# sgl-project/rbg

Hardware: NVIDIA B200
Metric: replica_x_node_affinity_scores_per_sec (higher is better)
Workload: dtype f32

## Files before the change

rbg_b200/csrc/plan_group.cuh:

```cuda
#pragma once
#include "select_fast.cuh"

namespace rbgtopo {

struct GroupTab {
  int* node;
  int* cons;
  float* aw;
  int mask, HT;
  int* cnt;
  int* dSlot;
  float* dBase;
  int* dFree;
  int* dAvail;
  int* dDom;
};
struct GroupRole {
  int count, demand, need, flags;
};

__host__ __device__ inline size_t group_smem_bytes(int QB, int PB, int HT, int CAP) {
  return (size_t)HT * 4 * (2 + QB) + (size_t)CAP * 20 +
         (size_t)PB * KS * (3 * 8 + 3 * 4) +
         (size_t)MAXP * 16 + (size_t)MAXP * RBGTOPO_MAX_GROUP_ROLES * 4;
}

__device__ __forceinline__ int gtab_insert(const GroupTab& T, int n) {
  int h = tab_hash(n, T.mask);
  while (true) {
    const int old = atomicCAS(&T.node[h], -1, n);
    if (old == -1) T.dSlot[atomicAdd(T.cnt, 1)] = h;
    if (old == -1 || old == n) return h;
    h = (h + 1) & T.mask;
  }
}
__device__ __forceinline__ bool gtab_has(const GroupTab& T, int n) {
  int h = tab_hash(n, T.mask);
  while (true) {
    const int k = T.node[h];
    if (k == n) return true;
    if (k == -1) return false;
    h = (h + 1) & T.mask;
  }
}
__device__ __forceinline__ float gtab_delta(const GroupTab& T, const float* pair_row, int Q, int slot) {
  float d = 0.0f;
  const float* aw = T.aw + slot;
  for (int q = 0; q < Q; ++q, aw += T.HT) d = fmaf(pair_row[q], *aw, d);
  return d;
}

#ifdef RBGTOPO_PHASE_CLOCKS
__device__ long long g_phase_clk[2048 * 32];
__device__ int g_dbg_skip;
__device__ long long g_cta_ns[2048 * 4];
__device__ __forceinline__ long long pg_gtime() { long long t; asm volatile("mov.u64 %0, %%globaltimer;" : "=l"(t)); return t; }
__device__ __forceinline__ int pg_smid() { int v; asm volatile("mov.u32 %0, %%smid;" : "=r"(v)); return v; }
#define PCLK(k) do { if (tid == 0 && blockIdx.x < 2048 && (k) < 32) g_phase_clk[blockIdx.x * 32 + (k)] = clock64(); } while (0)
#define PCLKL(k) do { if ((k) >= 0 && (threadIdx.x & 31) == 0 && blockIdx.x < 2048 && (k) < 32) g_phase_clk[blockIdx.x * 32 + (k)] = clock64(); } while (0)
#else
#define PCLK(k) do {} while (0)
#define PCLKL(k) do {} while (0)
#endif

struct BgCand {
  unsigned long long ob;
  int node, free_, owner, dom;
};
__device__ __forceinline__ BgCand bg_attrs(const TopoDev& t, int need_i, int i, int n_sel, unsigned long long ob) {
  BgCand c;
  c.ob = ob;
  c.node = -1;
  c.free_ = 0;
  c.owner = -1;
  c.dom = -1;
  if (i < n_sel) {
    c.node = need_i > 0 ? key_node(ob) : i;
    c.free_ = t.free_[c.node];
    c.owner = t.node_owner[c.node];
    c.dom = t.domain[c.node];
  }
  return c;
}
__device__ __forceinline__ BgCand bg_load(const TopoDev& t, int need_i, int i, int n_sel) {
  return bg_attrs(t, need_i, i, n_sel, (i < n_sel && need_i > 0) ? t.order_all[i] : 0ull);
}

__device__ __forceinline__ void select_role_group(const TopoDev& t, int gid, bool excl_step, const GroupRole& role,
                                                  const float* pair_row, int Q, int K, int dom, const GroupTab& T,
                                                  int cnt, bool have_first, const BgCand& first, int dbg,
                                                  unsigned long long* sAcc, int* sAccAv,
                                                  unsigned long long* sPat, int* sPatAv, unsigned long long* out,
                                                  int* outAvail) {
  const int lane = threadIdx.x & 31;
  if (dom == DOM_NONE || K <= 0) {
    out[lane] = 0;
    outAvail[lane] = 0;
    __syncwarp();
    return;
  }
  const int demand = role.demand;
  const float need = (float)role.need;
  const bool rexcl = excl_step && (role.flags & RBGTOPO_ROLE_EXCLUSIVE);

  constexpr int EREG = 8;
  auto entry_key = [&](int i) -> unsigned long long {
    const int av = T.dAvail[i], dd = T.dDom[i];
    if (av >= demand && !(rexcl && dd < 0) && (dom == DOM_ANY || (dd & 0x7FFFFFFF) == dom)) {
      const int slot = T.dSlot[i];
      return make_key(fmaf(need, T.dBase[i], gtab_delta(T, pair_row, Q, slot)), T.node[slot]);
    }
    return 0ull;
  };
  unsigned long long kreg[EREG];
#ifdef RBGTOPO_PHASE_CLOCKS
  if (g_dbg_skip & 2) cnt = 0;
#endif
#pragma unroll
  for (int j = 0; j < EREG; ++j) {
    kreg[j] = 0ull;
    if (32 * j < cnt) {
      const int i = lane + 32 * j;
      if (i < cnt) kreg[j] = entry_key(i);
    }
  }
  int npat = 0;
  {
    unsigned long long prev = ~0ull;
    for (; npat < K; ++npat) {
      unsigned long long best = 0;
      int bi = 0;
#pragma unroll
      for (int j = 0; j < EREG; ++j)
        if (32 * j < cnt && kreg[j] < prev && kreg[j] > best) { best = kreg[j]; bi = lane + 32 * j; }
      for (int i = lane + 32 * EREG; i < cnt; i += 32) {
        const unsigned long long k = entry_key(i);
        if (k < prev && k > best) { best = k; bi = i; }
      }
      const unsigned long long m = warp_max_u64(best);
      if (m == 0) break;
      if (best == m) { sPat[npat] = m; sPatAv[npat] = T.dAvail[bi]; }
      prev = m;
    }
  }
  __syncwarp();
  PCLKL(dbg);

  int acc = 0;
  for (int pos = 0; pos < t.n && acc < K; pos += 32) {
    const BgCand c = (pos == 0 && have_first) ? first : bg_load(t, role.need, pos + lane, t.n);
    bool ok = c.node >= 0 && c.free_ >= demand;
    if (ok && rexcl) ok = (c.owner == -1 || c.owner == gid);
    if (ok && dom != DOM_ANY) ok = c.dom == dom;
    if (ok) ok = !gtab_has(T, c.node);
    const uint32_t m = __ballot_sync(FULL, ok);
    const int idx = acc + __popc(m & ((1u << lane) - 1u));
    if (ok && idx < K) {
      const float base = __uint_as_float((uint32_t)(c.ob >> 32) ^ 0x80000000u);
      sAcc[idx] = role.need > 0 ? make_key(need * base, c.node) : make_key(0.0f, c.node);
      sAccAv[idx] = c.free_;
    }
    acc += __popc(m);
  }
  acc = min(acc, K);
  __syncwarp();
  PCLKL(dbg < 0 ? -1 : dbg + 1);

  merge_lists(sAcc, sAccAv, acc, sPat, sPatAv, npat, K, out, outAvail);
}

__device__ __forceinline__ void gtab_add_anchor(const TopoDev& t, const GroupTab& T, int m, int q, int c, int dem) {
  const int lane = threadIdx.x & 31;
  if (lane == 0 && dem > 0) atomicAdd(&T.cons[gtab_insert(T, m)], dem);
  if (c <= 0) return;
  const int rb = t.row_ptr[m], re = t.row_ptr[m + 1];
  for (int j = rb + lane; j <= re; j += 32) {
    int nn, wv;
    if (j < re) {
      nn = t.col[j];
      wv = t.w[j] * c;
    } else {
      nn = m;
      wv = RBGTOPO_SELF_W * c;
    }
    atomicAdd(&T.aw[(size_t)q * T.HT + gtab_insert(T, nn)], (float)wv);
  }
}

__device__ __forceinline__ int wave_next(const int* roles, int q, int& cr, int& taken, int* role, int* count) {
  while (cr < q && roles[4 * cr + 1] - taken <= 0) { ++cr; taken = 0; }
  if (cr >= q) return 0;
  const int level = roles[4 * cr];
  int n = 0, P = 0;
  while (cr < q && roles[4 * cr] == level && n < RBGTOPO_MAX_STEP_REPLICAS && P < RBGTOPO_MAX_STEP_ROLES) {
    const int left = roles[4 * cr + 1] - taken;
    if (left <= 0) { ++cr; taken = 0; continue; }
    const int take = min(left, RBGTOPO_MAX_STEP_REPLICAS - n);
    role[P] = cr;
    count[P] = take;
    ++P;
    n += take;
    taken += take;
    if (taken == roles[4 * cr + 1]) { ++cr; taken = 0; }
  }
  return P;
}

constexpr int RTAB_WARPS = 4;
__global__ void __launch_bounds__(32 * RTAB_WARPS) k_group_rtab(const int* __restrict__ grp, int words, int n_groups, int n_rows,
                                                              int2* __restrict__ rtab) {
  __shared__ int sR[RTAB_WARPS][4 * RBGTOPO_MAX_GROUP_ROLES], sP[RTAB_WARPS][RBGTOPO_MAX_GROUP_ROLES * RBGTOPO_MAX_GROUP_ROLES];
  __shared__ int sPl[RTAB_WARPS][RBGTOPO_MAX_GROUP_ROLES], sRole[RTAB_WARPS][RBGTOPO_MAX_STEP_ROLES], sCount[RTAB_WARPS][RBGTOPO_MAX_STEP_ROLES];
  __shared__ int sRec[RTAB_WARPS][RBGTOPO_MAX_STEP_ROLES], sNP[RTAB_WARPS];
  const int lane = threadIdx.x & 31, wi = threadIdx.x >> 5;
  const int g = blockIdx.x * RTAB_WARPS + wi;
  if (g >= n_groups) return;
  const int* rec = grp + RBGTOPO_HDR_WORDS + (size_t)g * RBGTOPO_GROUP_WORDS;
  const int gid = rec[0], q = rec[3];
  const long long roff = rec[4], poff = rec[5];
  const bool excl = (rec[1] & RBGTOPO_STEP_EXCLUSIVE) != 0;
  if (q < 1 || q > RBGTOPO_MAX_GROUP_ROLES || roff < 0 || roff + 4 * q > words || poff < 0 || poff + q * q > words) return;
  if (rec[9] <= 0) return;
  for (int i = lane; i < 4 * q; i += 32) sR[wi][i] = grp[roff + i];
  for (int i = lane; i < q * q; i += 32) sP[wi][i] = grp[poff + i];
  if (lane < RBGTOPO_MAX_GROUP_ROLES) sPl[wi][lane] = 0;
  __syncwarp();
  int cr = 0, tk = 0;
  long long row = rec[8];
  if (row < 0) return;
  while (row < n_rows) {
    if (lane == 0) sNP[wi] = wave_next(sR[wi], q, cr, tk, sRole[wi], sCount[wi]);
    __syncwarp();
    const int P = sNP[wi];
    if (P == 0) break;
    if (lane < P) {
      const int ri = sRole[wi][lane];
      int need = 0;
      for (int j = 0; j < q; ++j)
        if (sP[wi][ri * q + j] > 0) need += sR[wi][4 * j + 1] - sPl[wi][j];
      const bool rexcl = excl && (sR[wi][4 * ri + 3] & RBGTOPO_ROLE_EXCLUSIVE);
      sRec[wi][lane] = emit_pack_row(sR[wi][4 * ri + 2], max(0, min(need, RBGTOPO_NEED_CAP)), rexcl);
    }
    __syncwarp();
    for (int p = 0; p < P; ++p) {
      const int cnt = sCount[wi][p];
      const int2 rr = make_int2(sRec[wi][p], gid);
      if (lane < cnt && row + lane < n_rows) rtab[row + lane] = rr;
      row += cnt;
    }
    if (lane < P) sPl[wi][sRole[wi][lane]] += sCount[wi][lane];
    __syncwarp();
  }
}

template <bool DIRECT>
__global__ void __launch_bounds__(32 * MAXP, 4) k_plan_group(TopoDev t, BatchDev b, int QB, int HT, int CAP, int record) {
  extern __shared__ __align__(16) unsigned char pg_smem[];
  __shared__ int sTakenNode[KS], sTakenAmt[KS], sTakenRole[KS], sRowB[KS], sRowN[KS];
  __shared__ int sDstar, sCnt, sNew, sStatus, sAny, sCorrN;
  const int tid = threadIdx.x, warp = tid >> 5, lane = tid & 31, nthreads = blockDim.x, nwarps = nthreads >> 5;
  const int PB = nwarps;
  GroupTab T;
  T.node = reinterpret_cast<int*>(pg_smem);
  T.cons = T.node + HT;
  T.aw = reinterpret_cast<float*>(T.cons + HT);
  T.mask = HT - 1;
  T.HT = HT;
  T.cnt = &sCnt;
  T.dSlot = reinterpret_cast<int*>(T.aw + (size_t)QB * HT);
  T.dBase = reinterpret_cast<float*>(T.dSlot + CAP);
  T.dFree = reinterpret_cast<int*>(T.dBase + CAP);
  T.dAvail = T.dFree + CAP;
  T.dDom = T.dAvail + CAP;
  unsigned long long* sList = reinterpret_cast<unsigned long long*>(T.dDom + CAP);
  unsigned long long* sAcc = sList + (size_t)PB * KS;
  unsigned long long* sPat = sAcc + (size_t)PB * KS;
  int* sListAv = reinterpret_cast<int*>(sPat + (size_t)PB * KS);
  int* sAccAv = sListAv + (size_t)PB * KS;
  int* sPatAv = sAccAv + (size_t)PB * KS;
  GroupRole* sRole = reinterpret_cast<GroupRole*>(sPatAv + (size_t)PB * KS);
  float* sPair = reinterpret_cast<float*>(sRole + MAXP);

  if (record) pdl_launch_dependents();
  PCLK(30);
#ifdef RBGTOPO_PHASE_CLOCKS
  if (tid == 0 && blockIdx.x < 2048) { g_cta_ns[blockIdx.x * 4] = pg_gtime(); g_cta_ns[blockIdx.x * 4 + 3] = pg_smid(); }
#endif
  int wave_i = 0;
  int step = b.perm ? b.perm[blockIdx.x] : blockIdx.x;
  __shared__ int sGR[DIRECT ? 4 * RBGTOPO_MAX_GROUP_ROLES : 1];
  __shared__ int sGP[DIRECT ? RBGTOPO_MAX_GROUP_ROLES * RBGTOPO_MAX_GROUP_ROLES : 1];
  __shared__ int sPlaced[DIRECT ? RBGTOPO_MAX_GROUP_ROLES : 1];
  __shared__ int sWRole[DIRECT ? RBGTOPO_MAX_STEP_ROLES : 1], sWCount[DIRECT ? RBGTOPO_MAX_STEP_ROLES : 1];
  __shared__ int sWP, sWN, sCr, sTk;
  int g_rep0 = 0, g_pend = 0, g_i0 = 0, g_stat = 0, g_dom = -1;
  StepHdr h;
  if (DIRECT) {
    const int* rec = b.blob + RBGTOPO_HDR_WORDS + (size_t)step * RBGTOPO_GROUP_WORDS;
    h.gid = rec[0];
    h.flags = rec[1] & (RBGTOPO_STEP_EXCLUSIVE | RBGTOPO_STEP_GANG);
    h.fixed_domain = (rec[1] & RBGTOPO_STEP_EXCLUSIVE) ? rec[2] : -1;
    h.Q = rec[3];
    h.role_off = rec[4];
    h.pair_off = rec[5];
    h.n_anchors = rec[6];
    h.anchor_off = rec[7];
    h.i0 = 0;
    g_rep0 = rec[8];
    g_pend = rec[9];
    h.P = 0; h.R = 0; h.rep_off = g_rep0; h.rolerow_off = 0; h.next_step = 0; h.n_cons = 0; h.cons_off = 0;
  } else {
    h = load_hdr(b, step);
  }
  for (int i = tid; i < HT; i += nthreads) {
    T.node[i] = -1;
    T.cons[i] = 0;
  }
  for (int i = tid; i < QB * HT; i += nthreads) T.aw[i] = 0.0f;
  if (tid == 0) sCnt = 0;
  if (DIRECT) {
    for (int i = tid; i < 4 * h.Q; i += nthreads) sGR[i] = b.blob[h.role_off + i];
    for (int i = tid; i < h.Q * h.Q; i += nthreads) sGP[i] = b.blob[h.pair_off + i];
    if (tid < RBGTOPO_MAX_GROUP_ROLES) sPlaced[tid] = 0;
    if (tid == 0) { sCr = 0; sTk = 0; }
  }
  const bool excl_step = (h.flags & RBGTOPO_STEP_EXCLUSIVE) != 0;
  const bool gang = (h.flags & RBGTOPO_STEP_GANG) != 0;
  const int gid = h.gid, Q = h.Q;
  int fixed = excl_step ? h.fixed_domain : -1;
  g_dom = fixed;
  const size_t stride = (size_t)t.slab_stride;
  __syncthreads();

  {
    const int* anc = b.blob + h.anchor_off;
    for (int a = warp; a < h.n_anchors - h.i0; a += nwarps) gtab_add_anchor(t, T, anc[3 * a], anc[3 * a + 1], anc[3 * a + 2], 0);
  }
  int n_new = 0;
  int cnt_done = 0;

  while (true) {
    PCLK(wave_i * 8 + 0);
    const unsigned long long ob0 = lane < t.n ? t.order_all[lane] : 0ull;
    if (DIRECT) {
      if (tid == 0) {
        int cr = sCr, tk = sTk;
        const int P = wave_next(sGR, Q, cr, tk, sWRole, sWCount);
        int n = 0;
        for (int k = 0; k < P; ++k) n += sWCount[k];
        sCr = cr;
        sTk = tk;
        sWP = P;
        sWN = n;
      }
      __syncthreads();
      h.P = sWP;
      h.R = sWN;
      h.rep_off = g_rep0 + g_i0;
      if (h.P == 0) break;
      if (tid < h.P) {
        const int ri = sWRole[tid];
        int need = 0;
        for (int j = 0; j < Q; ++j)
          if (sGP[ri * Q + j] > 0) need += sGR[4 * j + 1] - sPlaced[j];
        sRole[tid] = GroupRole{sWCount[tid], sGR[4 * ri + 2], min(need, RBGTOPO_NEED_CAP), (sGR[4 * ri + 3] & 0xFF) | (ri << 8)};
      }
      for (int i = tid; i < h.P * Q; i += nthreads)
        sPair[(i / Q) * RBGTOPO_MAX_GROUP_ROLES + i % Q] = (float)sGP[sWRole[i / Q] * Q + i % Q];
    } else {
      if (tid < h.P) {
        const int4 r = *reinterpret_cast<const int4*>(b.blob + h.role_off + 4 * tid);
        sRole[tid] = GroupRole{r.x, r.y, r.z, r.w};
      }
      for (int i = tid; i < h.P * Q; i += nthreads)
        sPair[(i / Q) * RBGTOPO_MAX_GROUP_ROLES + i % Q] = (float)b.blob[h.pair_off + i];
    }
    if (tid == 0) sCorrN = 0;
    if (tid < n_new) {
      const int m = sTakenNode[tid];
      const int rb = t.row_ptr[m], re = t.row_ptr[m + 1];
      sRowB[tid] = rb;
      sRowN[tid] = re - rb + 1;
      atomicAdd(&T.cons[gtab_insert(T, m)], sTakenAmt[tid]);
    }
    __syncthreads();
    BgCand first;
    const bool have_first = warp < h.P;
    if (have_first) first = bg_attrs(t, sRole[warp].need, lane, t.n, ob0);
    {
      int total = 0;
      for (int a = 0; a < n_new; ++a) total += sRowN[a];
      for (int e = tid; e < total; e += nthreads) {
        int a = 0, off = e;
        while (off >= sRowN[a]) off -= sRowN[a++];
        const int m = sTakenNode[a], q = sTakenRole[a];
        int nn, wv;
        if (off < sRowN[a] - 1) {
          nn = t.col[sRowB[a] + off];
          wv = t.w[sRowB[a] + off];
        } else {
          nn = m;
          wv = RBGTOPO_SELF_W;
        }
        atomicAdd(&T.aw[(size_t)q * HT + gtab_insert(T, nn)], (float)wv);
      }
    }
    __syncthreads();
    PCLK(wave_i * 8 + 1);

    const int cnt = sCnt;
    for (int d = cnt_done + tid; d < cnt; d += nthreads) {
      const int node = T.node[T.dSlot[d]];
      int dd = t.domain[node];
      if (excl_step) {
        const int o = t.node_owner[node];
        if (!(o == -1 || o == gid)) dd |= 0x80000000;
      }
      T.dBase[d] = t.base[node];
      T.dFree[d] = t.free_[node];
      T.dDom[d] = dd;
    }
    cnt_done = cnt;
    __syncthreads();
    for (int d = tid; d < cnt; d += nthreads) T.dAvail[d] = T.dFree[d] - T.cons[T.dSlot[d]];
    __syncthreads();
    PCLK(wave_i * 8 + 2);

    PCLK(wave_i * 8 + 3);
    int dstar = excl_step ? fixed : -1;
    if (excl_step && fixed < 0) {
      int pstar = -1;
      for (int p = 0; p < h.P; ++p)
        if (sRole[p].flags & RBGTOPO_ROLE_EXCLUSIVE) { pstar = p; break; }
      if (warp == 0) {
        int d = -1;
        if (pstar >= 0) {
          select_role_group(t, gid, excl_step, sRole[pstar], sPair + pstar * RBGTOPO_MAX_GROUP_ROLES, Q, 1, DOM_ANY, T,
                            cnt, pstar == 0, first, 29, sAcc, sAccAv, sPat, sPatAv, sList, sListAv);
          const unsigned long long top = sList[0];
          d = top ? t.domain[key_node(top)] : -1;
        }
        if (lane == 0) sDstar = d;
      }
      __syncthreads();
      dstar = sDstar;
    }
    if (warp < h.P) {
      const int p = warp;
      const bool rexcl = excl_step && (sRole[p].flags & RBGTOPO_ROLE_EXCLUSIVE);
      const int dom = rexcl ? (dstar >= 0 ? dstar : DOM_NONE) : DOM_ANY;
      int K = 0;
      for (int q = 0; q <= p; ++q) K += sRole[q].count;
      K = min(K, t.n);
      select_role_group(t, gid, excl_step, sRole[p], sPair + p * RBGTOPO_MAX_GROUP_ROLES, Q, K, dom, T, cnt, true, first, warp == 0 ? wave_i * 8 + 6 : -1,
                        sAcc + p * KS, sAccAv + p * KS, sPat + p * KS, sPatAv + p * KS, sList + p * KS,
                        sListAv + p * KS);
      if (!DIRECT) b.merged[(size_t)(h.rolerow_off + p) * KS + lane] = sList[p * KS + lane];
    }
    __syncthreads();
    PCLK(wave_i * 8 + 4);

#ifdef RBGTOPO_PHASE_CLOCKS
    if (!(g_dbg_skip & 1))
#endif
    if (warp != 0 && record) {
      int* const reg = b.corr + (size_t)b.poff[step] * b.corr_w;
      for (int d = tid - 32; d < cnt; d += nthreads - 32) {
        const int slot = T.dSlot[d];
        const int node = T.node[slot];
        if (node < t.slab_lo || node >= t.slab_hi) continue;
        const int av = T.dAvail[d];
        const bool consumed = T.cons[slot] > 0;
        float v[MAXP];
        bool any = false;
#pragma unroll
        for (int p = 0; p < MAXP; ++p) {
          v[p] = 0.0f;
          if (p < h.P) {
            v[p] = (consumed && av < sRole[p].demand) ? -INFINITY
                                                      : gtab_delta(T, sPair + p * RBGTOPO_MAX_GROUP_ROLES, Q, slot);
            any |= v[p] != 0.0f;
          }
        }
        if (any) {
          int* e = reg + (size_t)atomicAdd(&sCorrN, 1) * b.corr_w;
          e[0] = node;
#pragma unroll
          for (int p = 0; p < MAXP; ++p)
            if (p < h.P) e[1 + p] = __float_as_int(v[p]);
        }
      }
    } else if (warp != 0) {
      if (wave_i == 0) {
        pdl_wait();
        pdl_launch_dependents();
      }
      float* const mrow0 = b.matrix + (size_t)h.rep_off * stride - t.slab_lo;
      for (int d = tid - 32; d < cnt; d += nthreads - 32) {
        const int slot = T.dSlot[d];
        const int node = T.node[slot];
        if (node < t.slab_lo || node >= t.slab_hi) continue;
        const int av = T.dAvail[d];
        const bool consumed = T.cons[slot] > 0;
        float* rowp = mrow0 + node;
        for (int p = 0; p < h.P; ++p) {
          const int count = sRole[p].count;
          if (consumed && av < sRole[p].demand) {
            for (int k = 0; k < count; ++k) rowp[(size_t)k * stride] = -INFINITY;
          } else {
            const float add = gtab_delta(T, sPair + p * RBGTOPO_MAX_GROUP_ROLES, Q, slot);
            if (add != 0.0f)
              for (int k = 0; k < count; ++k) sel_red_add_f32(rowp + (size_t)k * stride, add);
          }
          rowp += (size_t)count * stride;
        }
      }
    }

    if (warp == 0) {
      int tnode = -1, tamt = 0, trole = 0;
      int ntaken = 0, unplaced = 0, r = 0;
      for (int p = 0; p < h.P; ++p) {
        const int count = sRole[p].count, demand = sRole[p].demand;
        const int grole = (sRole[p].flags >> 8) & 0xFF;
        const unsigned long long key = sList[p * KS + lane];
        const int node = key ? key_node(key) : -1;
        const int av = sListAv[p * KS + lane];
        for (int c = 0; c < count; ++c, ++r) {
          int used = 0;
          for (int i = 0; i < ntaken; ++i) {
            const int n_i = __shfl_sync(FULL, tnode, i), a_i = __shfl_sync(FULL, tamt, i);
            used += n_i == node ? a_i : 0;
          }
          const uint32_t okm = __ballot_sync(FULL, key != 0 && av - used >= demand);
          const int pick = okm ? __shfl_sync(FULL, node, __ffs(okm) - 1) : -1;
          if (pick >= 0) {
            if (lane == ntaken) { tnode = pick; tamt = demand; trole = grole; }
            ++ntaken;
          } else {
            ++unplaced;
          }
          if (lane == 0) b.assign[h.rep_off + r] = pick;
        }
      }
      int status = unplaced ? RBGTOPO_PLACED_PART : RBGTOPO_PLACED_ALL;
      if (unplaced && gang) {
        status = RBGTOPO_GANG_FAILED;
        for (int i = lane; i < h.R; i += 32) b.assign[h.rep_off + i] = -1;
        ntaken = 0;
      }
      if (lane < ntaken) {
        sTakenNode[lane] = tnode;
        sTakenAmt[lane] = tamt;
        sTakenRole[lane] = trole;
      }
      if (lane == 0) {
        if (!DIRECT) {
          b.status[step] = status;
          b.domain_out[step] = dstar;
          b.dstar[step] = dstar;
        }
        sNew = ntaken;
        sStatus = status;
        sAny = ntaken > 0;
      }
    }
    if (DIRECT && tid < h.P) sPlaced[sWRole[tid]] += sWCount[tid];
    __syncthreads();
    if (record && tid == 0) b.corr_cnt[step] = sCorrN;
    PCLK(wave_i * 8 + 5);
    ++wave_i;
    if (DIRECT) {
      g_stat = max(g_stat, sStatus);
      if (dstar >= 0) g_dom = dstar;
      g_i0 += h.R;
      n_new = sNew;
      if (excl_step && dstar >= 0 && sAny) fixed = dstar;
      if (sStatus == RBGTOPO_GANG_FAILED) break;
      continue;
    }
    if (h.next_step <= 0) break;
    n_new = sNew;
    if (excl_step && dstar >= 0 && sAny) fixed = dstar;
    if (sStatus == RBGTOPO_GANG_FAILED) {
      if (warp == 0)
        for (int s2 = h.next_step; s2 > 0;) {
          const StepHdr h2 = load_hdr(b, s2);
          for (int i = lane; i < h2.R; i += 32) b.assign[h2.rep_off + i] = -1;
          if (lane == 0) {
            b.status[s2] = RBGTOPO_GANG_FAILED;
            b.domain_out[s2] = -1;
            b.dstar[s2] = -1;
            if (record) b.corr_cnt[s2] = 0;
          }
          s2 = h2.next_step;
        }
      break;
    }
    step = h.next_step;
    h = load_hdr(b, step);
  }
  if (DIRECT) {
    if (g_stat == RBGTOPO_GANG_FAILED || (gang && g_stat != RBGTOPO_PLACED_ALL)) {
      for (int i = tid; i < g_pend; i += nthreads) b.assign[g_rep0 + i] = -1;
      g_stat = RBGTOPO_GANG_FAILED;
      g_dom = -1;
    }
    if (tid == 0) {
      b.status[step] = g_stat;
      b.domain_out[step] = excl_step ? g_dom : -1;
    }
  }
  PCLK(31);
#ifdef RBGTOPO_PHASE_CLOCKS
  if (tid == 0 && blockIdx.x < 2048) { g_cta_ns[blockIdx.x * 4 + 1] = pg_gtime(); g_cta_ns[blockIdx.x * 4 + 2] = sCnt; }
#endif
}

constexpr int CORRECT_WARPS = 4;
__global__ void __launch_bounds__(32 * CORRECT_WARPS) k_plan_correct(TopoDev t, BatchDev b) {
  const int lane = threadIdx.x & 31;
  const int step = blockIdx.x * CORRECT_WARPS + (threadIdx.x >> 5);
  if (step >= b.n_steps) return;
  const int cnt = b.corr_cnt[step];
  if (cnt <= 0) return;
  const int* __restrict__ hdr = b.blob + RBGTOPO_HDR_WORDS + (size_t)step * RBGTOPO_STEP_WORDS;
  const int P = hdr[3], role_off = hdr[4], rep_off = hdr[12];
  const int my_count = lane < P ? b.blob[role_off + 4 * lane] : 0;
  const size_t stride = (size_t)t.slab_stride;
  float* const mrow0 = b.matrix + (size_t)rep_off * stride - t.slab_lo;
  const int* const reg = b.corr + (size_t)b.poff[step] * b.corr_w;
  for (int e0 = 0; e0 < cnt; e0 += 32) {
    const int e = e0 + lane;
    const int* rec = reg + (size_t)e * b.corr_w;
    float* rowp = e < cnt ? mrow0 + rec[0] : nullptr;
    for (int p = 0; p < P; ++p) {
      const int count = __shfl_sync(FULL, my_count, p);
      if (e < cnt) {
        const float v = __int_as_float(rec[1 + p]);
        if (v == -INFINITY) {
          for (int k = 0; k < count; ++k) rowp[(size_t)k * stride] = -INFINITY;
        } else if (v != 0.0f) {
          for (int k = 0; k < count; ++k) sel_red_add_f32(rowp + (size_t)k * stride, v);
        }
        rowp += (size_t)count * stride;
      }
    }
  }
}

}
```

rbg_b200/csrc/select.cuh:

```cuda
#pragma once
#include "kernels.cuh"
#include "p2p.cuh"

namespace rbgtopo {

constexpr int DOM_ANY = -2;
constexpr int DOM_NONE = -1;

constexpr int STEP_SKIP = 4;
constexpr int SEL_CORRECT = 1;
constexpr int SEL_CHAIN = 2;

struct StepHdr {
  int gid, flags, fixed_domain, P, role_off, Q, pair_off, n_anchors, anchor_off, n_cons, cons_off, R, rep_off,
      rolerow_off, next_step, i0;
};
__device__ __forceinline__ StepHdr load_hdr(const BatchDev& b, int step) {
  const int* hdr = b.blob + RBGTOPO_HDR_WORDS + (size_t)step * RBGTOPO_STEP_WORDS;
  StepHdr h;
  h.gid = hdr[0]; h.flags = hdr[1]; h.fixed_domain = hdr[2]; h.P = hdr[3]; h.role_off = hdr[4];
  h.Q = hdr[5]; h.pair_off = hdr[6]; h.n_anchors = hdr[7]; h.anchor_off = hdr[8];
  h.n_cons = hdr[9]; h.cons_off = hdr[10]; h.R = hdr[11]; h.rep_off = hdr[12]; h.rolerow_off = hdr[13];
  h.next_step = hdr[14]; h.i0 = hdr[15];
  return h;
}
__device__ __forceinline__ int role_k(const BatchDev& b, const StepHdr& h, int p, int n) {
  int k = 0;
  for (int q = 0; q <= p; ++q) k += b.blob[h.role_off + 4 * q];
  return min(k, n);
}
__device__ __forceinline__ int role_rowbase(const BatchDev& b, const StepHdr& h, int p) {
  int k = 0;
  for (int q = 0; q < p; ++q) k += b.blob[h.role_off + 4 * q];
  return k;
}

__device__ __forceinline__ void build_candidates(const TopoDev& t, const BatchDev& b, const StepHdr& h,
                                                 int* cand, int* sCnt) {
  const int lane = threadIdx.x & 31, warp = threadIdx.x >> 5, nwarps = blockDim.x >> 5;
  const int* anc = b.blob + h.anchor_off;
  for (int a = warp; a < h.n_anchors; a += nwarps) {
    const int m = anc[3 * a];
    const int rb = t.row_ptr[m], re = t.row_ptr[m + 1];
    for (int j0 = rb; j0 <= re; j0 += 32) {
      const int j = j0 + lane;
      int nn = -1;
      if (j < re) nn = t.col[j];
      else if (j == re) nn = m;
      const bool keep = nn >= t.slab_lo && nn < t.slab_hi;
      const uint32_t msk = __ballot_sync(FULL, keep);
      int base = 0;
      if (lane == 0 && msk) base = atomicAdd(sCnt, __popc(msk));
      base = __shfl_sync(FULL, base, 0);
      if (keep) cand[base + __popc(msk & ((1u << lane) - 1u))] = nn;
    }
  }
  const int* con = b.blob + h.cons_off;
  for (int c = threadIdx.x; c < h.n_cons; c += blockDim.x) {
    const int m = con[2 * c];
    if (m >= t.slab_lo && m < t.slab_hi) cand[atomicAdd(sCnt, 1)] = m;
  }
}

__device__ __forceinline__ void sel_red_add_f32(float* p, float v) {
  asm volatile("red.global.add.f32 [%0], %1;" ::"l"(p), "f"(v) : "memory");
}

__device__ __forceinline__ void correct_step(const TopoDev& t, const BatchDev& b, const StepHdr& h) {
  const int lane = threadIdx.x & 31, warp = threadIdx.x >> 5, nwarps = blockDim.x >> 5;
  const size_t stride = (size_t)t.slab_stride;
  float* const mrow0 = b.matrix + (size_t)h.rep_off * stride - t.slab_lo;
  const int* con = b.blob + h.cons_off;
  for (int c = threadIdx.x; c < h.n_cons; c += blockDim.x) {
    const int m = con[2 * c];
    if (m >= t.slab_lo && m < t.slab_hi && con[2 * c + 1] > 0) {
      int amt = 0;
      for (int k = 0; k < h.n_cons; ++k)
        if (con[2 * k] == m) amt += con[2 * k + 1];
      const int avail = t.free_[m] - amt;
      float* rowp = mrow0 + m;
      for (int p = 0; p < h.P; ++p) {
        const int count = b.blob[h.role_off + 4 * p], demand = b.blob[h.role_off + 4 * p + 1];
        if (avail < demand)
          for (int k = 0; k < count; ++k) rowp[(size_t)k * stride] = -INFINITY;
        rowp += (size_t)count * stride;
      }
    }
  }
  const int* anc = b.blob + h.anchor_off;
  for (int a = warp; a < h.n_anchors; a += nwarps) {
    const int m = anc[3 * a], q = anc[3 * a + 1], c = anc[3 * a + 2];
    if (c == 0) continue;
    const int rb = t.row_ptr[m], re = t.row_ptr[m + 1];
    for (int j = rb + lane; j <= re; j += 32) {
      int nn, wv;
      if (j < re) {
        nn = t.col[j];
        wv = t.w[j] * c;
      } else {
        nn = m;
        wv = RBGTOPO_SELF_W * c;
      }
      if (nn >= t.slab_lo && nn < t.slab_hi) {
        float* rowp = mrow0 + nn;
        for (int p = 0; p < h.P; ++p) {
          const int count = b.blob[h.role_off + 4 * p];
          const int coef = b.blob[h.pair_off + p * h.Q + q];
          if (coef) {
            const float add = (float)(coef * wv);
            for (int k = 0; k < count; ++k) sel_red_add_f32(rowp + (size_t)k * stride, add);
          }
          rowp += (size_t)count * stride;
        }
      }
    }
  }
}

__device__ __forceinline__ void select_role(const TopoDev& t, const BatchDev& b, const StepHdr& h, int p,
                                            int K, int dom, const int* cand, int cnt,
                                            unsigned long long* kcache, int kcap,
                                            unsigned long long* sAcc, unsigned long long* sPat,
                                            unsigned long long* out) {
  const int lane = threadIdx.x & 31;
  if (dom == DOM_NONE || K <= 0) {
    out[lane] = 0;
    return;
  }
  const int demand = b.blob[h.role_off + 4 * p + 1];
  const int need_i = b.blob[h.role_off + 4 * p + 2];
  const bool rexcl = (h.flags & RBGTOPO_STEP_EXCLUSIVE) && (b.blob[h.role_off + 4 * p + 3] & RBGTOPO_ROLE_EXCLUSIVE);
  const float* __restrict__ row =
      b.matrix + (size_t)(h.rep_off + role_rowbase(b, h, p)) * t.slab_stride - t.slab_lo;

  int npat = 0;
  {
    const bool cached = kcache != nullptr && cnt <= kcap;
    if (cached) {
      for (int i = lane; i < cnt; i += 32) {
        const int node = cand[i];
        const float x = row[node];
        kcache[i] = (x != -INFINITY && (dom == DOM_ANY || t.domain[node] == dom)) ? make_key(x, node) : 0ull;
      }
      __syncwarp();
    }
    unsigned long long prev = ~0ull;
    for (; npat < K; ++npat) {
      unsigned long long best = 0;
      if (cached) {
        for (int i = lane; i < cnt; i += 32) {
          const unsigned long long k = kcache[i];
          if (k < prev && k > best) best = k;
        }
      } else {
        for (int i = lane; i < cnt; i += 32) {
          const int node = cand[i];
          const float x = row[node];
          if (x != -INFINITY && (dom == DOM_ANY || t.domain[node] == dom)) {
            const unsigned long long k = make_key(x, node);
            if (k < prev && k > best) best = k;
          }
        }
      }
      best = warp_max_u64(best);
      if (best == 0) break;
      if (lane == 0) sPat[npat] = best;
      prev = best;
    }
  }

  const int slab_len = t.slab_hi - t.slab_lo;
  const float need = (float)need_i;
  int acc = 0;
  for (int pos = 0; pos < slab_len && acc < K; pos += 32) {
    const int i = pos + lane;
    int node = -1;
    unsigned long long key = 0;
    bool ok = false;
    if (i < slab_len) {
      if (need_i > 0) {
        const unsigned long long ob = t.order[i];
        node = key_node(ob);
        const float base = __uint_as_float((uint32_t)(ob >> 32) ^ 0x80000000u);
        key = make_key(need * base, node);
      } else {
        node = t.slab_lo + i;
        key = make_key(0.0f, node);
      }
      ok = t.free_[node] >= demand;
      if (ok && rexcl) {
        const int o = t.node_owner[node];
        ok = (o == -1 || o == h.gid);
      }
      if (ok && dom != DOM_ANY) ok = t.domain[node] == dom;
    }
    if (__any_sync(FULL, ok)) {
      for (int e = 0; e < cnt; ++e)
        if (cand[e] == node) ok = false;
    }
    const uint32_t m = __ballot_sync(FULL, ok);
    const int idx = acc + __popc(m & ((1u << lane) - 1u));
    if (ok && idx < K) sAcc[idx] = key;
    acc += __popc(m);
  }
  acc = min(acc, K);
  __syncwarp();

  if (lane == 0) {
    int ia = 0, ip = 0;
    for (int r = 0; r < KS; ++r) {
      unsigned long long v = 0;
      if (r < K) {
        const unsigned long long a = ia < acc ? sAcc[ia] : 0ull;
        const unsigned long long c = ip < npat ? sPat[ip] : 0ull;
        if (a > c) { v = a; ++ia; } else if (c) { v = c; ++ip; }
      }
      out[r] = v;
    }
  }
  __syncwarp();
}

__device__ __forceinline__ void chain_step(const BatchDev& b, const StepHdr& h, int status, int dstar) {
  const int lane = threadIdx.x & 31;
  __syncwarp();
  int* wb = const_cast<int*>(b.blob);
  const bool excl = (h.flags & RBGTOPO_STEP_EXCLUSIVE) != 0;
  const bool dead = status == RBGTOPO_GANG_FAILED;
  bool any = false;
  for (int i = 0; i < h.R; ++i) any |= b.assign[h.rep_off + i] >= 0;
  const int fixed = excl ? ((dstar >= 0 && any) ? dstar : h.fixed_domain) : -1;
  for (int s2 = h.next_step; s2 > 0;) {
    int* hd = wb + RBGTOPO_HDR_WORDS + (size_t)s2 * RBGTOPO_STEP_WORDS;
    const int n_static = hd[7] - hd[15];
    int rr = 0;
    for (int p = 0; p < h.P; ++p) {
      const int count = b.blob[h.role_off + 4 * p], demand = b.blob[h.role_off + 4 * p + 1];
      const int q = (b.blob[h.role_off + 4 * p + 3] >> 8) & 0xFF;
      for (int c = lane; c < count; c += 32) {
        const int node = b.assign[h.rep_off + rr + c];
        int* ar = wb + hd[8] + 3 * (n_static + h.i0 + rr + c);
        int* cr = wb + hd[10] + 2 * (h.i0 + rr + c);
        ar[0] = node >= 0 ? node : 0;
        ar[1] = q;
        ar[2] = node >= 0 ? 1 : 0;
        cr[0] = node >= 0 ? node : 0;
        cr[1] = node >= 0 ? demand : 0;
      }
      rr += count;
    }
    const int nxt = hd[14];
    if (lane == 0) {
      hd[2] = fixed;
      hd[1] = dead ? (hd[1] | STEP_SKIP) : (hd[1] & ~STEP_SKIP);
    }
    s2 = nxt;
  }
}

__device__ __forceinline__ void greedy_step(const TopoDev& t, const BatchDev& b, int step, const StepHdr& h,
                                            const unsigned long long (*sList)[KS], int* sTakenNode,
                                            int* sTakenAmt, int dstar, bool chain = false) {
  const int lane = threadIdx.x & 31;
  const int* con = b.blob + h.cons_off;
  int ntaken = 0, unplaced = 0, r = 0;
  for (int p = 0; p < h.P; ++p) {
    const int count = b.blob[h.role_off + 4 * p], demand = b.blob[h.role_off + 4 * p + 1];
    for (int c = 0; c < count; ++c, ++r) {
      int pick = -1;
      for (int k = 0; k < KS; ++k) {
        const unsigned long long key = sList[p][k];
        if (key == 0) break;
        const int node = key_node(key);
        int used = 0;
        for (int i = lane; i < h.n_cons; i += 32)
          if (con[2 * i] == node) used += con[2 * i + 1];
        for (int i = lane; i < ntaken; i += 32)
          if (sTakenNode[i] == node) used += sTakenAmt[i];
        used = __reduce_add_sync(FULL, used);
        if (t.free_[node] - used >= demand) {
          pick = node;
          break;
        }
      }
      if (pick >= 0) {
        if (lane == 0) {
          sTakenNode[ntaken] = pick;
          sTakenAmt[ntaken] = demand;
        }
        ++ntaken;
        __syncwarp();
      } else {
        ++unplaced;
      }
      if (lane == 0) b.assign[h.rep_off + r] = pick;
    }
  }
  __syncwarp();
  int status = unplaced ? RBGTOPO_PLACED_PART : RBGTOPO_PLACED_ALL;
  if (unplaced && (h.flags & RBGTOPO_STEP_GANG)) {
    status = RBGTOPO_GANG_FAILED;
    for (int i = lane; i < h.R; i += 32) b.assign[h.rep_off + i] = -1;
  }
  if (lane == 0) {
    b.status[step] = status;
    b.domain_out[step] = dstar;
    b.dstar[step] = dstar;
  }
  if (chain && h.next_step > 0) chain_step(b, h, status, dstar);
}

constexpr int CAND_CAP = 512;
__host__ __device__ inline size_t select_smem_bytes(int PB) { return (size_t)CAND_CAP * 4 + (size_t)PB * CAND_CAP * 8; }

struct CandRef { const int* p; int cnt; };
__device__ __forceinline__ CandRef stage_candidates(const TopoDev& t, const BatchDev& b, int step, const StepHdr& h,
                                                    int* sCand, int* sCnt) {
  const int cap = b.poff[step + 1] - b.poff[step];
  int* dst = cap <= CAND_CAP ? sCand : b.cand + b.poff[step];
  if (threadIdx.x == 0) *sCnt = 0;
  __syncthreads();
  build_candidates(t, b, h, dst, sCnt);
  __syncthreads();
  CandRef r;
  r.p = dst;
  r.cnt = *sCnt;
  return r;
}

__global__ void __launch_bounds__(32 * MAXP) k_select_assign(TopoDev t, BatchDev b, int step_begin, int mode) {
  extern __shared__ __align__(16) unsigned char sel_smem[];
  int* sCand = reinterpret_cast<int*>(sel_smem);
  unsigned long long* sKeys = reinterpret_cast<unsigned long long*>(sel_smem + (size_t)CAND_CAP * 4);
  __shared__ unsigned long long sList[MAXP][KS];
  __shared__ unsigned long long sAcc[MAXP][KS];
  __shared__ unsigned long long sPat[MAXP][KS];
  __shared__ int sTakenNode[KS], sTakenAmt[KS];
  __shared__ int sDstar, sCnt;
  const int warp = threadIdx.x >> 5, lane = threadIdx.x & 31;
  const int step = step_begin + blockIdx.x;
  const StepHdr h = load_hdr(b, step);
  const bool excl_step = (h.flags & RBGTOPO_STEP_EXCLUSIVE) != 0;
  if (h.flags & STEP_SKIP) {
    if (warp == 0) {
      for (int i = lane; i < h.R; i += 32) b.assign[h.rep_off + i] = -1;
      if (lane == 0) {
        b.status[step] = RBGTOPO_GANG_FAILED;
        b.domain_out[step] = -1;
        b.dstar[step] = -1;
      }
    }
    return;
  }
  if (mode & SEL_CORRECT) {
    correct_step(t, b, h);
    __threadfence();
  }
  const CandRef cr = stage_candidates(t, b, step, h, sCand, &sCnt);
  const int* cand = cr.p;
  const int cnt = cr.cnt;
  int dstar = excl_step ? h.fixed_domain : -1;
  if (excl_step && h.fixed_domain < 0) {
    int pstar = -1;
    for (int p = 0; p < h.P; ++p)
      if (b.blob[h.role_off + 4 * p + 3] & RBGTOPO_ROLE_EXCLUSIVE) { pstar = p; break; }
    if (warp == 0) {
      int d = -1;
      if (pstar >= 0) {
        select_role(t, b, h, pstar, 1, DOM_ANY, cand, cnt, sKeys, CAND_CAP, sAcc[0], sPat[0], sList[0]);
        const unsigned long long top = sList[0][0];
        d = top ? t.domain[key_node(top)] : -1;
      }
      if (lane == 0) sDstar = d;
    }
    __syncthreads();
    dstar = sDstar;
  }
  if (warp < h.P) {
    const int p = warp;
    const bool rexcl = excl_step && (b.blob[h.role_off + 4 * p + 3] & RBGTOPO_ROLE_EXCLUSIVE);
    const int dom = rexcl ? (dstar >= 0 ? dstar : DOM_NONE) : DOM_ANY;
    select_role(t, b, h, p, role_k(b, h, p, t.n), dom, cand, cnt, sKeys + (size_t)p * CAND_CAP, CAND_CAP, sAcc[p],
                sPat[p], sList[p]);
    b.merged[(size_t)(h.rolerow_off + p) * KS + lane] = sList[p][lane];
  }
  __syncthreads();
  if (warp == 0) greedy_step(t, b, step, h, sList, sTakenNode, sTakenAmt, dstar, (mode & SEL_CHAIN) != 0);
}

__global__ void __launch_bounds__(32 * MAXP) k_select(TopoDev t, BatchDev b, int pass2) {
  extern __shared__ __align__(16) unsigned char sel_smem[];
  int* sCand = reinterpret_cast<int*>(sel_smem);
  unsigned long long* sKeys = reinterpret_cast<unsigned long long*>(sel_smem + (size_t)CAND_CAP * 4);
  __shared__ unsigned long long sAcc[MAXP][KS];
  __shared__ unsigned long long sPat[MAXP][KS];
  __shared__ int sCnt;
  const int warp = threadIdx.x >> 5;
  const int step = blockIdx.x;
  const StepHdr h = load_hdr(b, step);
  const bool excl_step = (h.flags & RBGTOPO_STEP_EXCLUSIVE) != 0;
  const bool unknown = excl_step && h.fixed_domain < 0;
  if (pass2 && !unknown) return;
  const CandRef cr = stage_candidates(t, b, step, h, sCand, &sCnt);
  const int* cand = cr.p;
  const int cnt = cr.cnt;
  if (warp >= h.P) return;
  const int p = warp;
  const bool rexcl = excl_step && (b.blob[h.role_off + 4 * p + 3] & RBGTOPO_ROLE_EXCLUSIVE);
  const int K = role_k(b, h, p, t.n);
  if (!pass2) {
    const int dom = (rexcl && !unknown) ? h.fixed_domain : DOM_ANY;
    select_role(t, b, h, p, K, dom, cand, cnt, sKeys + (size_t)p * CAND_CAP, CAND_CAP, sAcc[p], sPat[p],
                b.lists + (size_t)(h.rolerow_off + p) * KS);
  } else if (rexcl) {
    const int d = b.dstar[step];
    select_role(t, b, h, p, K, d >= 0 ? d : DOM_NONE, cand, cnt, sKeys + (size_t)p * CAND_CAP, CAND_CAP, sAcc[p],
                sPat[p], b.excl + (size_t)(h.rolerow_off + p) * KS);
  }
}

constexpr int SEL_WARPS = 4;
constexpr int SEL_THREADS = SEL_WARPS * 32;

__device__ __forceinline__ int merge_parts(const unsigned long long* src, long long stride, int parts, int K,
                                           unsigned long long* out ) {
  const int lane = threadIdx.x & 31;
  unsigned long long prev = ~0ull;
  int r = 0;
  for (; r < K; ++r) {
    unsigned long long best = 0;
    for (int i = lane; i < parts * K; i += 32) {
      const unsigned long long k = src[(long long)(i / K) * stride + (i % K)];
      if (k < prev && k > best) best = k;
    }
    best = warp_max_u64(best);
    if (best == 0) break;
    if (lane == 0) out[r] = best;
    prev = best;
  }
  for (int q = r + lane; q < KS; q += 32) out[q] = 0;
  __syncwarp();
  return r;
}

__global__ void __launch_bounds__(SEL_THREADS) k_merge(TopoDev t, BatchDev b, int step_begin, int count, P2PWait pw) {
  p2p_wait_cta(pw);
  const int warp = threadIdx.x >> 5, lane = threadIdx.x & 31;
  const int idx = blockIdx.x * SEL_WARPS + warp;
  if (idx >= count) return;
  const int step = step_begin + idx;
  const StepHdr h = load_hdr(b, step);
  const bool excl_step = (h.flags & RBGTOPO_STEP_EXCLUSIVE) != 0;
  int dstar = excl_step ? h.fixed_domain : -1;
  bool dstar_set = !excl_step || h.fixed_domain >= 0;
  for (int p = 0; p < h.P; ++p) {
    unsigned long long* out = b.merged + (size_t)(h.rolerow_off + p) * KS;
    merge_parts(b.lists_all + (size_t)(h.rolerow_off + p) * KS, b.part_stride, b.parts, role_k(b, h, p, t.n), out);
    if (!dstar_set && (b.blob[h.role_off + 4 * p + 3] & RBGTOPO_ROLE_EXCLUSIVE)) {
      const unsigned long long top = out[0];
      dstar = top ? t.domain[key_node(top)] : -1;
      dstar_set = true;
    }
  }
  if (lane == 0) b.dstar[step] = dstar;
}

__global__ void __launch_bounds__(SEL_THREADS) k_greedy(TopoDev t, BatchDev b, int step_begin, int count, int chain, P2PWait pw) {
  p2p_wait_cta(pw);
  __shared__ unsigned long long sList[SEL_WARPS][MAXP][KS];
  __shared__ int sTakenNode[SEL_WARPS][KS];
  __shared__ int sTakenAmt[SEL_WARPS][KS];
  const int warp = threadIdx.x >> 5, lane = threadIdx.x & 31;
  const int idx = blockIdx.x * SEL_WARPS + warp;
  if (idx >= count) return;
  const int step = step_begin + idx;
  const StepHdr h = load_hdr(b, step);
  if (h.flags & STEP_SKIP) {
    for (int i = lane; i < h.R; i += 32) b.assign[h.rep_off + i] = -1;
    if (lane == 0) {
      b.status[step] = RBGTOPO_GANG_FAILED;
      b.domain_out[step] = -1;
    }
    return;
  }
  const bool unknown = (h.flags & RBGTOPO_STEP_EXCLUSIVE) && h.fixed_domain < 0;
  for (int p = 0; p < h.P; ++p) {
    const bool rexcl = (b.blob[h.role_off + 4 * p + 3] & RBGTOPO_ROLE_EXCLUSIVE) != 0;
    unsigned long long* mg = b.merged + (size_t)(h.rolerow_off + p) * KS;
    if (unknown && rexcl)
      merge_parts(b.excl_all + (size_t)(h.rolerow_off + p) * KS, b.excl_part_stride, b.parts,
                  role_k(b, h, p, t.n), mg);
    sList[warp][p][lane] = mg[lane];
  }
  __syncwarp();
  greedy_step(t, b, step, h, sList[warp], sTakenNode[warp], sTakenAmt[warp], b.dstar[step], chain != 0);
}

}
```

Before: 1080 billion.

## Prefetch next step header, roles and pair weights into shared memory during current wave

After: 1076 billion, median of 6. No clear change (-0.4%).

```diff
diff --git a/rbg_b200/csrc/plan_group.cuh b/rbg_b200/csrc/plan_group.cuh
--- a/rbg_b200/csrc/plan_group.cuh
+++ b/rbg_b200/csrc/plan_group.cuh
@@ -293,7 +293,11 @@
   __shared__ int sPlaced[DIRECT ? RBGTOPO_MAX_GROUP_ROLES : 1];
   __shared__ int sWRole[DIRECT ? RBGTOPO_MAX_STEP_ROLES : 1], sWCount[DIRECT ? RBGTOPO_MAX_STEP_ROLES : 1];
   __shared__ int sWP, sWN, sCr, sTk;
+  __shared__ int sNH[DIRECT ? 1 : 2][DIRECT ? 1 : RBGTOPO_STEP_WORDS];
+  __shared__ GroupRole sNRole[DIRECT ? 1 : MAXP];
+  __shared__ float sNPair[DIRECT ? 1 : MAXP * RBGTOPO_MAX_GROUP_ROLES];
   int g_rep0 = 0, g_pend = 0, g_i0 = 0, g_stat = 0, g_dom = -1;
+  const unsigned long long ob0 = lane < t.n ? t.order_all[lane] : 0ull;
   StepHdr h;
   if (DIRECT) {
     const int* rec = b.blob + RBGTOPO_HDR_WORDS + (size_t)step * RBGTOPO_GROUP_WORDS;
@@ -332,6 +336,13 @@
   const size_t stride = (size_t)t.slab_stride;
   __syncthreads();
 
+  if (!DIRECT && tid >= nthreads - 32) {
+    if (lane < h.P) {
+      const int4 r = *reinterpret_cast<const int4*>(b.blob + h.role_off + 4 * lane);
+      sRole[lane] = GroupRole{r.x, r.y, r.z, r.w};
+    }
+    for (int i = lane; i < h.P * Q; i += 32) sPair[(i / Q) * RBGTOPO_MAX_GROUP_ROLES + i % Q] = (float)b.blob[h.pair_off + i];
+  }
   {
     const int* anc = b.blob + h.anchor_off;
     for (int a = warp; a < h.n_anchors - h.i0; a += nwarps) gtab_add_anchor(t, T, anc[3 * a], anc[3 * a + 1], anc[3 * a + 2], 0);
@@ -341,7 +352,6 @@
 
   while (true) {
     PCLK(wave_i * 8 + 0);
-    const unsigned long long ob0 = lane < t.n ? t.order_all[lane] : 0ull;
     if (DIRECT) {
       if (tid == 0) {
         int cr = sCr, tk = sTk;
@@ -368,12 +378,12 @@
       for (int i = tid; i < h.P * Q; i += nthreads)
         sPair[(i / Q) * RBGTOPO_MAX_GROUP_ROLES + i % Q] = (float)sGP[sWRole[i / Q] * Q + i % Q];
     } else {
-      if (tid < h.P) {
-        const int4 r = *reinterpret_cast<const int4*>(b.blob + h.role_off + 4 * tid);
-        sRole[tid] = GroupRole{r.x, r.y, r.z, r.w};
-      }
-      for (int i = tid; i < h.P * Q; i += nthreads)
-        sPair[(i / Q) * RBGTOPO_MAX_GROUP_ROLES + i % Q] = (float)b.blob[h.pair_off + i];
+      if (wave_i > 0) {
+        if (tid < h.P) sRole[tid] = sNRole[tid];
+        for (int i = tid; i < h.P * RBGTOPO_MAX_GROUP_ROLES; i += nthreads) sPair[i] = sNPair[i];
+      }
+      if (h.next_step > 0 && tid >= nthreads - 32 && lane < RBGTOPO_STEP_WORDS)
+        sNH[wave_i & 1][lane] = b.blob[RBGTOPO_HDR_WORDS + (size_t)h.next_step * RBGTOPO_STEP_WORDS + lane];
     }
     if (tid == 0) sCorrN = 0;
     if (tid < n_new) {
@@ -384,6 +394,15 @@
       atomicAdd(&T.cons[gtab_insert(T, m)], sTakenAmt[tid]);
     }
     __syncthreads();
+    if (!DIRECT && h.next_step > 0 && tid >= nthreads - 32) {
+      const int* nh = sNH[wave_i & 1];
+      const int nP = nh[3], nQ = nh[5];
+      if (lane < nP) {
+        const int4 r = *reinterpret_cast<const int4*>(b.blob + nh[4] + 4 * lane);
+        sNRole[lane] = GroupRole{r.x, r.y, r.z, r.w};
+      }
+      for (int i = lane; i < nP * nQ; i += 32) sNPair[(i / nQ) * RBGTOPO_MAX_GROUP_ROLES + i % nQ] = (float)b.blob[nh[6] + i];
+    }
     BgCand first;
     const bool have_first = warp < h.P;
     if (have_first) first = bg_attrs(t, sRole[warp].need, lane, t.n, ob0);
@@ -598,7 +617,7 @@
       break;
     }
     step = h.next_step;
-    h = load_hdr(b, step);
+    h = load_hdr(sNH[(wave_i - 1) & 1]);
   }
   if (DIRECT) {
     if (g_stat == RBGTOPO_GANG_FAILED || (gang && g_stat != RBGTOPO_PLACED_ALL)) {
diff --git a/rbg_b200/csrc/select.cuh b/rbg_b200/csrc/select.cuh
--- a/rbg_b200/csrc/select.cuh
+++ b/rbg_b200/csrc/select.cuh
@@ -15,14 +15,16 @@
   int gid, flags, fixed_domain, P, role_off, Q, pair_off, n_anchors, anchor_off, n_cons, cons_off, R, rep_off,
       rolerow_off, next_step, i0;
 };
-__device__ __forceinline__ StepHdr load_hdr(const BatchDev& b, int step) {
-  const int* hdr = b.blob + RBGTOPO_HDR_WORDS + (size_t)step * RBGTOPO_STEP_WORDS;
+__device__ __forceinline__ StepHdr load_hdr(const int* hdr) {
   StepHdr h;
   h.gid = hdr[0]; h.flags = hdr[1]; h.fixed_domain = hdr[2]; h.P = hdr[3]; h.role_off = hdr[4];
   h.Q = hdr[5]; h.pair_off = hdr[6]; h.n_anchors = hdr[7]; h.anchor_off = hdr[8];
   h.n_cons = hdr[9]; h.cons_off = hdr[10]; h.R = hdr[11]; h.rep_off = hdr[12]; h.rolerow_off = hdr[13];
   h.next_step = hdr[14]; h.i0 = hdr[15];
   return h;
+}
+__device__ __forceinline__ StepHdr load_hdr(const BatchDev& b, int step) {
+  return load_hdr(b.blob + RBGTOPO_HDR_WORDS + (size_t)step * RBGTOPO_STEP_WORDS);
 }
 __device__ __forceinline__ int role_k(const BatchDev& b, const StepHdr& h, int p, int n) {
   int k = 0;
```
